# yatpor/bpc_baseline

Measured on AMD Instinct MI355X. Metric: detection-pairs matched/sec, higher is better.
Workload: dtype f64

## Files before the change

### bpc_baseline_amd/_native.py

```python
from __future__ import annotations

import ctypes
import os
import re

PKG_DIR = os.path.dirname(os.path.abspath(__file__))
LIB_PATH = os.environ.get("MVM_LIB_PATH") or os.path.join(PKG_DIR, "lib", "libmvmatch.so")
HEADER_PATH = os.path.join(os.path.dirname(PKG_DIR), "include", "mvmatch.h")

MVM_OK = 0
MVM_MAX_CAMS = 8
MVM_MAX_PAIRS = 28
MVM_F32, MVM_F64 = 0, 1

PAIRWISE_ARGMIN = {"default": 0, "lazy_transposed": 1, "lazy_rows": 2, "eager": 3}
CUBE_KERNEL = {"default": 0, "small": 1, "fused": 2, "workspace": 3, "generic": 4}


class MvmOptions(ctypes.Structure):
    _fields_ = [(n, ctypes.c_int32) for n in (
        "size", "pairwise_argmin", "pairwise_rows_per_wave", "pairwise_row_groups",
        "cube_kernel", "cube_rows_per_instr", "lsap_wave_max_cols", "lsap_multi_g",
        "lsap_lds_max_cols", "lsap_lds_small_cols", "lsap_mid_max_cols", "lsap_reg_max_cols",
        "lsap_reg_threads", "lsap_mreg_max_cols", "pairwise_row_interleave",
        "cube_cols_per_lane", "pairwise_xcd_fronts", "lsap_sparse_min_cols",
        "lsap_sparse_blocks", "cube_tile_rows")]


OPTION_FIELDS = [n for n, _ in MvmOptions._fields_[1:]]


def make_options(**kw):
    if not kw:
        return None
    o = MvmOptions()
    o.size = ctypes.sizeof(MvmOptions)
    for k, v in kw.items():
        if k not in OPTION_FIELDS:
            raise ValueError(f"unknown mvm_options field {k!r}")
        if k == "pairwise_argmin" and isinstance(v, str):
            v = PAIRWISE_ARGMIN[v]
        if k == "cube_kernel" and isinstance(v, str):
            v = CUBE_KERNEL[v]
        setattr(o, k, int(v))
    return o


class MvmError(RuntimeError):

    def __init__(self, fn: str, status: int, message: str):
        super().__init__(f"{fn} failed with status {status}: {message}")
        self.status = status


_vp = ctypes.c_void_p
_i32 = ctypes.c_int32
_i64 = ctypes.c_int64
_sz = ctypes.c_size_t

SIGNATURES = {
    "mvm_version": (ctypes.c_char_p, []),
    "mvm_last_error_string": (ctypes.c_char_p, []),
    "mvm_status_string": (ctypes.c_char_p, [ctypes.c_int]),
    "mvm_options_init": (None, [_vp]),
    "mvm_pairwise_residual_argmin": (ctypes.c_int, [
        _vp, _vp, _vp, _vp, _vp,
        _i32, _i32, _i32, _i32,
        _vp, _vp, _vp, _vp, _vp,
        _vp]),
    "mvm_pairwise_residual_argmin_ex": (ctypes.c_int, [
        _vp, _vp, _vp, _vp, _vp,
        _i32, _i32, _i32, _i32,
        _vp, _vp, _vp, _vp, _vp,
        _vp, _vp]),
    "mvm_pairwise_residual_argmin_pitched": (ctypes.c_int, [
        _vp, _vp, _vp, _vp, _vp,
        _i32, _i32, _i32, _i32, _i32,
        _vp, _vp, _vp, _vp, _vp,
        _vp, _vp]),
    "mvm_pairwise_residual_f64": (ctypes.c_int, [
        _vp, _vp, _vp, _vp, _vp,
        _i32, _i32, _i32, _i32,
        _i64, _i64, _vp,
        _vp]),
    "mvm_triplet_workspace_bytes": (_sz, [_i32, _i32]),
    "mvm_triplet_cost_argmin": (ctypes.c_int, [
        _vp, _vp, _vp, _i32, _i32,
        _vp, _vp, _vp, _vp, _vp,
        _vp, _sz, _vp]),
    "mvm_triplet_cost_argmin_ex": (ctypes.c_int, [
        _vp, _vp, _vp, _i32, _i32,
        _vp, _vp, _vp, _vp, _vp,
        _vp, _sz, _vp, _vp]),
    "mvm_triplet_cost_argmin_bmin8": (ctypes.c_int, [
        _vp, _vp, _vp, _i32, _i32,
        _vp, _vp, _vp, _vp, _vp,
        _vp, _vp,
        _vp, _sz, _vp, _vp]),
    "mvm_triplet_minima": (ctypes.c_int, [
        _vp, _vp, _vp, _i32, _i32,
        _vp, _vp, _vp, _vp,
        _vp, _sz, _vp, _vp]),
    "mvm_lsap_plan": (_i64, [_i32, _vp, _vp, _vp, _vp]),
    "mvm_lsap_plan_ex": (_i64, [_i32, _vp, _vp, _i32, _vp, _vp]),
    "mvm_lsap_solve": (ctypes.c_int, [
        _vp, _vp, _vp, _i32, _vp, _vp,
        _vp, _sz, _vp, _vp, _vp, _vp]),
    "mvm_lsap_solve_bounded": (ctypes.c_int, [
        _vp, _vp, _vp, _i32, _vp, _vp,
        _vp, _sz, _vp, _vp, _vp,
        _i64, _i64, _vp]),
    "mvm_lsap_solve_ex": (ctypes.c_int, [
        _vp, _i32, _vp, _vp, _i32, _vp, _vp,
        _vp, _sz, _vp, _vp, _vp,
        _i64, _i64, _vp, _vp]),
    "mvm_lsap_solve_ex2": (ctypes.c_int, [
        _vp, _i32, _vp, _vp, _i32, _vp, _vp,
        _vp, _sz, _vp, _vp, _vp,
        _i64, _i64, _i64, _vp, _vp]),
    "mvm_lsap_solve_ex3": (ctypes.c_int, [
        _vp, _i32, _vp, _vp, _i32, _vp, _vp,
        _vp, _sz, _vp, _vp, _vp,
        _i64, _i64, _i64,
        _vp, _vp, _vp, _vp, _vp]),
    "mvm_lsap_plan_resid": (_i64, [_i32, _vp, _vp, _vp, _vp]),
    "mvm_lsap_sparse_bounds": (None, [_vp, _vp, _vp]),
    "mvm_lsap_sparse_stats_offset": (_i64, [_i64, _i64]),
    "mvm_lsap_solve_resid": (ctypes.c_int, [
        _vp, _i32, _vp, _vp,
        _vp, _sz, _vp, _vp, _vp,
        _i64, _i64, _i64,
        _vp, _vp, _vp, _vp, _vp,
        _vp, _i32, _vp, _vp]),
    "mvm_pack_detections": (ctypes.c_int, [
        _vp, _vp, _vp, _vp, _i32,
        ctypes.c_float, ctypes.c_float,
        _vp, _vp, _vp, _vp, _vp, _vp]),
    "mvm_triangulate_dlt": (ctypes.c_int, [
        _vp, _vp, _vp, _i32, _i32, _vp, _vp]),
    "mvm_select_triangulate": (ctypes.c_int, [
        _vp, _vp, _vp, _vp, _vp, _vp,
        _vp, _vp, _i32, ctypes.c_double,
        _vp, _vp, _vp, _vp, _vp]),
    "mvm_select_triangulate_resid": (ctypes.c_int, [
        _vp, _i32, _vp, _vp, _vp, _vp,
        _vp, _vp, _i32, ctypes.c_double,
        _vp, _vp, _vp, _vp, _vp]),
    "mvm_compact_matches": (ctypes.c_int, [
        _vp, _vp, _vp, _vp, _vp,
        _vp, _vp, _vp, _i32, _i32,
        _vp, _vp, _vp, _vp, _vp, _vp, _vp,
        _vp]),
    "mvm_rig_matrices": (ctypes.c_int, [
        _vp, _vp, _vp, _vp,
        _i32, _i32, _i32,
        _vp, _vp, _vp, _vp]),
    "mvm_hbm_write_probe": (ctypes.c_int, [_vp, _sz, _vp]),
}

_lib = None


def header_symbols() -> list:
    with open(HEADER_PATH) as fh:
        text = fh.read()
    return re.findall(r"^\s*(?:const\s+)?[a-z_0-9]+\s*\*?\s*(mvm_[a-z_0-9]+)\s*\(", text, re.M)


def load(path: str = LIB_PATH):
    global _lib
    if _lib is not None:
        return _lib
    if not os.path.exists(path):
        raise ImportError(
            f"{path} not found: build the HIP library first "
            "(python -c 'import __graft_entry__ as g; g.build()')")
    lib = ctypes.CDLL(path)
    for name, (res, args) in SIGNATURES.items():
        fn = getattr(lib, name)
        fn.restype = res
# ... 14 lines not shown
```

### bpc_baseline_amd/csrc/mvm_lsap_sparse.h

```cpp
#pragma once

#include <hip/hip_runtime.h>
#include <stdint.h>

#include "mvmatch.h"

constexpr int kSpMaxCols = 65536;
constexpr int kSpMaxShort = 1024;
constexpr int kSpBlock = 32;
constexpr int kSpTB = 16;
constexpr int kSpLCap = 128;
constexpr int kSpTileCols = 2048;
constexpr int kSparseMinCols = 4096;
constexpr int kWaveMaxCols = 1024;

struct LsapIo {
    const void *cost;
    const int64_t *cost_offs;
    const int64_t *dims;
    const int64_t *ws_offs;
    unsigned char *ws;
    const int64_t *out_offs;
    int64_t *row_ind;
    int64_t *col_ind;
    int32_t *status;
};

struct LsapSparseArgs : LsapIo {
    int32_t lo;
    int32_t wave_max;
    int32_t s_cap;
    const uint16_t *bmin8;
    const int64_t *bmin8_offs;
    const int64_t *segs;
    int32_t tb;
    const double *resid = nullptr;
    int64_t resid_stride = 0;
    int32_t resid_ld = 0;
    int32_t resid_rows = 0;
    const uint16_t *bm32 = nullptr;
    const int64_t *bm32_offs = nullptr;
};

constexpr int32_t kSpStatusBounds = 4;

constexpr int kSpMaxBlocks = 2048;

__host__ __device__ inline int lsap_sparse_seg(const LsapSparseArgs &a, int p, bool tr, int L) {
    if (((!a.bmin8 || !a.bmin8_offs) && !a.bm32) || !a.segs || !tr) return 0;
    const int64_t seg = a.segs[p];
    if (seg <= 0 || L % seg != 0) return 0;
    return (L / seg) * ((seg + 31) / 32) <= kSpMaxBlocks ? (int)seg : 0;
}

__host__ __device__ inline bool lsap_sparse_class(int32_t lo, int32_t wave_max, int64_t R, int64_t K) {
    const int64_t lng = R > K ? R : K, sht = R > K ? K : R;
    return lo > 0 && lng >= lo && lng > wave_max && lng <= kSpMaxCols && sht >= 1 && sht <= kSpMaxShort;
}

struct SpLayout {
    size_t stats, flags, bm, lcol, lval, ln, theta, total;
};
constexpr int kSpStats = 4;

__host__ __device__ inline SpLayout lsap_sparse_layout(int64_t S, int64_t L, size_t elem, bool tr,
                                                       bool ext_bm = false) {
    SpLayout y;
    size_t o = 0;
    auto take = [&](size_t bytes) {
        const size_t at = o;
        o += (bytes + 255) & ~(size_t)255;
        return at;
    };
    const int64_t nbf = (L + kSpBlock - 1) / kSpBlock, nbs = L < kSpMaxBlocks ? L : kSpMaxBlocks;
    const int64_t nb = tr && nbs > nbf ? nbs : nbf;
    const int64_t nt = (L + kSpTileCols - 1) / kSpTileCols;
    y.stats = take(kSpStats * 4);
    y.flags = take((size_t)(nt > 32 ? nt : 32) * 4);
    y.bm = take(ext_bm ? 0 : (size_t)S * nb * elem);
    y.lcol = take((size_t)S * kSpLCap * 4);
    y.lval = take((size_t)S * kSpLCap * elem);
    y.ln = take((size_t)S * 4);
    y.theta = take((size_t)S * elem);
    y.total = o;
    return y;
}

int lsap_sparse_launch_f32(const LsapSparseArgs &a, int32_t n, int64_t long_max, hipStream_t s);
int lsap_sparse_launch_f64(const LsapSparseArgs &a, int32_t n, int64_t long_max, hipStream_t s);
```

### bpc_baseline_amd/csrc/mvm_lsap_sparse.hip

```cpp
#include "mvm_lsap_sparse.h"

#include <math.h>
#include <stdint.h>

#include "mvm_device.h"
#include "mvm_internal.h"

#pragma clang fp contract(off)

namespace {

constexpr int kSpNT = 256;
constexpr int kSpRowGroups = 16;

template <typename CT>
struct SpKey;
template <>
struct SpKey<float> {
    using T = uint32_t;
    static constexpr T kMax = 0xFFFFFFFFu;
    __device__ static T of(float x) {
        const uint32_t b = __float_as_uint(x + 0.0f);
        return (b & 0x80000000u) ? ~b : (b | 0x80000000u);
    }
// ... 461 lines not shown
                if (c) {
                    const int pos = ng + sp_mbcnt(m);
                    if (pos < kSpLCap) s_grp[wave][pos] = e;
                }
                ng += __popcll(m);
            }
            __builtin_amdgcn_wave_barrier();
            nent = ng;
            eshift = 3;
            ent = s_grp[wave];
        }
        int cnt = kSpLCap + 1;
        if (nent <= kSpLCap) {
            cnt = 0;
            const int per = kWaveLanes >> eshift, emask = (1 << eshift) - 1;
            for (int m0 = 0; m0 < nent; m0 += 8 * per) {
                CT val[8];
                int col[8];
#pragma unroll
                for (int u = 0; u < 8; ++u) {
                    const int idx = m0 + u * per + (lane >> eshift);
                    const int cb = idx < nent ? ent[idx] : 0;
                    const int j = (cb & 0xFFFF) + (lane & emask);
                    col[u] = (lane & emask) < (cb >> 16) ? j : -1;
                    val[u] = col[u] >= 0 ? src.at(s, j) : (CT)0;
                }
#pragma unroll
                for (int u = 0; u < 8; ++u) {
                    const bool keep = col[u] >= 0 && val[u] <= theta;
                    const uint64_t m = __ballot(keep);
                    if (keep) {
                        const int pos = cnt + sp_mbcnt(m);
                        if (pos < kSpLCap) {
                            lcol[(int64_t)s * kSpLCap + pos] = col[u];
                            lval[(int64_t)s * kSpLCap + pos] = val[u];
                        }
                    }
                    cnt += __popcll(m);
                }
            }
        }
        __builtin_amdgcn_wave_barrier();
        if (lane == 0) {
            ln[s] = cnt <= kSpLCap ? cnt : -1;
            theta_out[s] = theta;
        }
    }
    if (ext) {
        bad = __syncthreads_or(bad);
        if (threadIdx.x == 0) reinterpret_cast<int32_t *>(ws + y.flags)[grp] = bad;
    }
}


struct SpRec {
    double a;
    double f;
    int32_t a_pos;
    int32_t a_q;
    int32_t a_ps;
    int32_t f_any;
    int32_t tail_q;
    uint32_t f_key;
};

__host__ __device__ inline size_t sp_solve_lds_bytes(int lw, int cap) {
    return (size_t)2 * lw * 4 + (size_t)8 * (cap + 4 * (cap + 1)) + (size_t)4 * (3 * cap + 5 * (cap + 1));
}

template <typename CT>
__device__ __forceinline__ double sp_block_min(double x, double *s_red, int wave) {
    x = wave_min_f64(x);
    if ((threadIdx.x & 63) == 0) s_red[wave] = x;
    __syncthreads();
    const double r = fmin(fmin(s_red[0], s_red[1]), fmin(s_red[2], s_red[3]));
    __syncthreads();
    return r;
}

__device__ __forceinline__ long long sp_block_max_i64(long long x, long long *s_red, int wave) {
    x = sp_wave_max_i64(x);
    if ((threadIdx.x & 63) == 0) s_red[wave] = x;
    __syncthreads();
    long long r = s_red[0];
    for (int w = 1; w < kSpNT / 64; ++w) r = s_red[w] > r ? s_red[w] : r;
    __syncthreads();
    return r;
}

template <typename CT, int KS>
__global__ __launch_bounds__(kSpNT) __attribute__((amdgpu_waves_per_eu(KS == 1 ? 4 : 1))) void sp_solve_kernel(LsapSparseArgs a, int32_t n, int32_t lw) {
    __shared__ SpRec s_rec[2][kSpNT / 64];
    __shared__ double s_redd[kSpNT / 64];
    __shared__ long long s_redl[kSpNT / 64];
    extern __shared__ __attribute__((aligned(16))) unsigned char s_dyn[];
    const int p = blockIdx.x;
    if (p >= n) return;
    const int64_t R = a.dims[2 * p], Kd = a.dims[2 * p + 1];
    if (R == 0 || Kd == 0) {
        if (threadIdx.x == 0) a.status[p] = 0;
        return;
    }
    if (!lsap_sparse_class(a.lo, a.wave_max, R, Kd)) {
        if (a.resid && threadIdx.x == 0) a.status[p] = kSpStatusBounds;
        return;
    }
    const bool tr = Kd < R;
    const int S = (int)(tr ? Kd : R), L = (int)(tr ? R : Kd);
    const int cap = a.s_cap;
    bool src_ok;
    const SpSrc<CT> src = sp_src<CT>(a, p, tr, S, L, lsap_sparse_seg(a, p, tr, L), src_ok);
    if (S > cap || L > 32 * lw || (KS == 1 && S > kSpNT) || !src_ok) {
        if (threadIdx.x == 0) a.status[p] = kSpStatusBounds;
        return;
    }
    const SpLayout y = lsap_sparse_layout(S, L, sizeof(CT), tr, a.bm32 != nullptr);
    const unsigned char *ws = a.ws + a.ws_offs[p];
    const int32_t *lcol = reinterpret_cast<const int32_t *>(ws + y.lcol);
    const CT *lval = reinterpret_cast<const CT *>(ws + y.lval);
    const int32_t *ln = reinterpret_cast<const int32_t *>(ws + y.ln);
    const CT *theta = reinterpret_cast<const CT *>(ws + y.theta);
    const int t = threadIdx.x, lane = t & 63, wave = t >> 6;

    uint32_t *s_asg = reinterpret_cast<uint32_t *>(s_dyn);
    uint32_t *s_mvb = s_asg + lw;
    double *s_u = reinterpret_cast<double *>(s_mvb + lw);
    double *s_m = s_u + cap;
    double *s_mp = s_m + cap + 1;
    double *s_f = s_mp + cap + 1;
    double *s_rb = s_f + cap + 1;
    int32_t *s_c4r = reinterpret_cast<int32_t *>(s_rb + cap + 1);
    int32_t *s_r4c = s_c4r + cap;
    int32_t *s_col = s_r4c + cap;
    int32_t *s_i = s_col + cap;
    int32_t *s_sl = s_i + cap + 1;
    int32_t *s_ps = s_sl + cap + 1;
    int32_t *s_mvc = s_ps + cap + 1;
    int32_t *s_mvp = s_mvc + cap + 1;

    {
        const int seg = lsap_sparse_seg(a, p, tr, L);
        const int nt = a.bm32 ? kSpRowGroups
                       : seg  ? ((L / seg) * ((seg + kSpBlock - 1) / kSpBlock) + 63) / 64
                              : (L + kSpTileCols - 1) / kSpTileCols;
        const int32_t *fl = reinterpret_cast<const int32_t *>(ws + y.flags);
        int bad = 0;
        for (int x = t; x < nt; x += kSpNT) bad |= fl[x];
        if (__syncthreads_or(bad)) {
            if (t == 0) a.status[p] = 1;
            return;
        }
    }
    __shared__ int s_novf;
    if (t == 0) s_novf = 0;
    int n_dense_min = 0, n_dense_tie = 0, n_steps = 0;
    for (int x = t; x < lw; x += kSpNT) {
        s_asg[x] = 0u;
        s_mvb[x] = 0u;
    }
    __syncthreads();
    {
        int ovf = 0;
// ... 334 lines not shown
                const int q = kk == k ? na : s_sl[kk];
                s_c4r[i2] = q;
                s_r4c[q] = i2;
                if (s == 0) break;
                kk = s - 1;
            }
        }
        __syncthreads();
    }
    if (t == 0) {
        int32_t *stt = reinterpret_cast<int32_t *>(a.ws + a.ws_offs[p] + y.stats);
        stt[0] = n_dense_min;
        stt[1] = n_dense_tie;
        stt[2] = s_novf;
        stt[3] = n_steps;
    }
    const int64_t o = a.out_offs[p];
    if (tr) {
        for (int kk = t; kk < S; kk += kSpNT) {
            const int rk = s_col[s_c4r[kk]];
            int rank = 0;
            for (int k2 = 0; k2 < S; ++k2) rank += s_col[s_c4r[k2]] < rk;
            a.row_ind[o + rank] = rk;
            a.col_ind[o + rank] = kk;
        }
    } else {
        for (int kk = t; kk < S; kk += kSpNT) {
            a.row_ind[o + kk] = kk;
            a.col_ind[o + kk] = s_col[s_c4r[kk]];
        }
    }
    if (t == 0) a.status[p] = 0;
}

template <typename CT>
int sp_launch(const LsapSparseArgs &a0, int32_t n, int64_t long_max, hipStream_t s) {
    LsapSparseArgs a = a0;
    const int64_t lmax = long_max < kSpMaxCols ? long_max : kSpMaxCols;
    const int tpp = (int)((lmax + kSpTileCols - 1) / kSpTileCols);
    if ((int64_t)n * tpp * kSpNT > 0xFFFFFFFFLL || (int64_t)n * kSpRowGroups * kSpNT > 0xFFFFFFFFLL ||
        (int64_t)n * (kSpMaxBlocks / 64) * kSpNT > 0xFFFFFFFFLL)
        return mvm_fail(MVM_ERR_UNSUPPORTED, "%d problems in one batch: split it", (int)n);
    if (sizeof(CT) != sizeof(float)) {
        a.bmin8 = nullptr;
        a.bmin8_offs = nullptr;
        a.segs = nullptr;
        a.resid = nullptr;
        a.bm32 = nullptr;
        a.bm32_offs = nullptr;
    }
    if (!a.resid) sp_blockmin_kernel<CT><<<dim3((unsigned)(n * tpp)), dim3(kSpNT), 0, s>>>(a, n, tpp);
    if (a.bmin8 && !a.bm32)
        sp_bmin8_reduce_kernel<<<dim3((unsigned)(n * (kSpMaxBlocks / 64))), dim3(kSpNT), 0, s>>>(a, n);
    if (sizeof(CT) == 4 && a.bm32)
        sp_lists_kernel<CT, sizeof(CT) == 4><<<dim3((unsigned)(n * kSpRowGroups)), dim3(kSpNT), 0, s>>>(a, n);
    else
        sp_lists_kernel<CT, false><<<dim3((unsigned)(n * kSpRowGroups)), dim3(kSpNT), 0, s>>>(a, n);
    const int cap = a.s_cap;
    const int lw = (int)(((lmax + 63) / 64) * 2);
    const size_t lds = sp_solve_lds_bytes(lw, cap);
    void (*kern)(LsapSparseArgs, int32_t, int32_t) = cap <= kSpNT ? sp_solve_kernel<CT, 1> : sp_solve_kernel<CT, 4>;
    if (const int st = mvm_raise_dynamic_lds(reinterpret_cast<const void *>(kern), lds)) return st;
    kern<<<dim3((unsigned)n), dim3(kSpNT), lds, s>>>(a, n, lw);
    return mvm_check_launch("lsap_sparse");
}

}

int lsap_sparse_launch_f32(const LsapSparseArgs &a, int32_t n, int64_t long_max, hipStream_t s) {
    return sp_launch<float>(a, n, long_max, s);
}

int lsap_sparse_launch_f64(const LsapSparseArgs &a, int32_t n, int64_t long_max, hipStream_t s) {
    return sp_launch<double>(a, n, long_max, s);
}

extern "C" {

int64_t mvm_lsap_sparse_stats_offset(int64_t rows, int64_t cols) {
    const bool tr = cols < rows;
    return (int64_t)lsap_sparse_layout(tr ? cols : rows, tr ? rows : cols, sizeof(float), tr).stats;
}

void mvm_lsap_sparse_bounds(int32_t *min_cols, int32_t *max_cols, int32_t *max_short) {
    if (min_cols) *min_cols = kSparseMinCols;
    if (max_cols) *max_cols = kSpMaxCols;
    if (max_short) *max_short = kSpMaxShort;
}

int64_t mvm_lsap_plan_resid(int32_t n_problems, const int64_t *rows, const int64_t *cols,
                            int64_t *ws_offs, int64_t *out_offs) {
    if (n_problems < 0 || (n_problems > 0 && (!rows || !cols || !ws_offs || !out_offs))) {
        mvm_set_error("mvm_lsap_plan_resid: invalid arguments");
        return -1;
    }
    const auto need = [](int64_t nr, int64_t nc, bool tr, size_t elem) {
        if (nc > kSpMaxCols || nr > kSpMaxShort) return (int64_t)0;
        return (int64_t)lsap_sparse_layout(nr, nc, elem, tr, true).total;
    };
    return mvm_lsap_plan_offsets("mvm_lsap_plan_resid", n_problems, rows, cols, sizeof(float), need,
                                 ws_offs, out_offs);
}

int mvm_lsap_solve_resid(const int64_t *dims_dev, int32_t n_problems, const int64_t *ws_offs_dev,
                         const int64_t *out_offs_dev, void *workspace_dev, size_t workspace_bytes,
                         int64_t *row_ind_dev, int64_t *col_ind_dev, int32_t *status_dev,
                         int64_t long_min, int64_t long_max, int64_t short_max,
                         const uint16_t *bmin8_dev, const int64_t *bmin8_offs_dev,
                         const uint16_t *bm32_dev, const int64_t *bm32_offs_dev,
                         const int64_t *segs_dev, const double *resid_dev, int32_t max_n,
                         const mvm_options *opts, mvm_stream_t stream) {
    mvm_clear_error();
    mvm_options o;
    int st = mvm_resolve_options(opts, o);
    if (st) return st;
    if (o.lsap_sparse_blocks < 0 || o.lsap_sparse_blocks > 64)
        return mvm_fail(MVM_ERR_INVALID_ARGUMENT, "lsap_sparse_blocks %d not in 0..64",
                        (int)o.lsap_sparse_blocks);
    if (n_problems < 0) return mvm_fail(MVM_ERR_INVALID_ARGUMENT, "negative n_problems");
    if (n_problems == 0) return MVM_OK;
    if (!dims_dev || !ws_offs_dev || !out_offs_dev || !status_dev)
        return mvm_fail(MVM_ERR_INVALID_ARGUMENT, "null pointer");
    const bool data_null = (bmin8_dev && !bmin8_offs_dev) || !bm32_dev || !bm32_offs_dev || !segs_dev ||
                           !resid_dev || !workspace_dev || !row_ind_dev || !col_ind_dev;
    if (max_n < 0 || max_n > kChunk)
        return mvm_fail(MVM_ERR_UNSUPPORTED, "mvm_lsap_solve_resid: views of at most %d detections "
                        "(max_n %d)", kChunk, (int)max_n);
    const int sp_lo = mvm_resolve_limit(o.lsap_sparse_min_cols, kSparseMinCols, INT32_MAX);
    const int wave_max = mvm_resolve_limit(o.lsap_wave_max_cols, kWaveMaxCols, kWaveMaxCols);
    if (long_max >= 1) {
        if (sp_lo <= 0 || long_min < sp_lo || long_min <= wave_max || long_max > kSpMaxCols ||
            short_max < 1 || short_max > kSpMaxShort)
            return mvm_fail(MVM_ERR_INVALID_ARGUMENT,
                            "mvm_lsap_solve_resid: long sides [%lld, %lld] / short sides <= %lld are not "
                            "all of the candidate-list class (long sides >= %d, > %d, <= %d; short sides "
                            "<= %d)", (long long)long_min, (long long)long_max, (long long)short_max, sp_lo,
                            wave_max, kSpMaxCols, kSpMaxShort);
        if (data_null) return mvm_fail(MVM_ERR_INVALID_ARGUMENT, "null pointer");
    }
    (void)workspace_bytes;
    LsapSparseArgs sa{};
    sa.dims = dims_dev;
    sa.ws_offs = ws_offs_dev;
    sa.ws = reinterpret_cast<unsigned char *>(workspace_dev);
    sa.out_offs = out_offs_dev;
    sa.row_ind = row_ind_dev;
    sa.col_ind = col_ind_dev;
    sa.status = status_dev;
    sa.lo = sp_lo > 0 ? sp_lo : 1;
    sa.wave_max = wave_max;
    sa.s_cap = (int32_t)(short_max < 1 ? 1 : short_max);
    sa.bmin8 = bmin8_dev;
    sa.bmin8_offs = bmin8_dev ? bmin8_offs_dev : nullptr;
    sa.segs = segs_dev;
    sa.tb = o.lsap_sparse_blocks ? o.lsap_sparse_blocks : kSpTB;
    const int ld = (max_n + 3) / 4 * 4;
    sa.resid = resid_dev;
    sa.resid_ld = ld;
    sa.resid_rows = max_n;
    sa.resid_stride = (int64_t)3 * max_n * ld;
    sa.bm32 = bm32_dev;
    sa.bm32_offs = bm32_offs_dev;
    return sp_launch<float>(sa, n_problems, long_max < 1 ? 1 : long_max,
                            reinterpret_cast<hipStream_t>(stream));
}

}
```

### bpc_baseline_amd/ops.py

```python
from __future__ import annotations

import ctypes
from typing import List, Optional, Tuple

import numpy as np
import torch
from torch import Tensor

from . import _native

__all__ = [
    "PairwisePlan", "TripletPlan",
    "pairwise_residual_argmin", "pairwise_residual_f64", "triplet_cost_argmin",
    "hbm_write_probe", "LsapPlan", "linear_sum_assignment_batched",
    "pack_detections", "triangulate_dlt", "select_triangulate",
    "triplet_minima", "linear_sum_assignment_resid", "select_triangulate_resid",
    "cube_free_scenes", "sparse_class_bounds", "lsap_sparse_stats", "compact_matches",
    "rig_matrices",
]


def _h2d_int64(arrays: List[np.ndarray], device: torch.device) -> List[Tensor]:
    flat = np.concatenate([np.ascontiguousarray(a, dtype=np.int64).reshape(-1) for a in arrays])
    host = torch.from_numpy(flat)
    if device.type == "cuda":
        dev = host.pin_memory().to(device, non_blocking=True)
    else:
        dev = host.to(device)
    out, o = [], 0
    for a in arrays:
        out.append(dev[o:o + a.size])
        o += a.size
    return out


def _opts_list(options: Optional[dict]) -> Optional[List[int]]:
    o = _native.make_options(**(options or {}))
    return None if o is None else [int(getattr(o, n)) for n in _native.OPTION_FIELDS]


def _opts_ref(opts: Optional[List[int]]):
    if opts is None:
        return None
    if len(opts) != len(_native.OPTION_FIELDS):
        raise ValueError(f"opts: expected {len(_native.OPTION_FIELDS)} values, got {len(opts)}")
    return ctypes.byref(_native.make_options(**dict(zip(_native.OPTION_FIELDS, opts))))


def _p(t: Optional[Tensor]):
    if t is None or t.numel() == 0:
        return None
    return ctypes.c_void_p(t.data_ptr())


def _stream(t: Tensor):
    return ctypes.c_void_p(torch.cuda.current_stream(t.device).cuda_stream)


def _require(t: Tensor, name: str, dtype: torch.dtype, device: torch.device) -> None:
    if t.dtype != dtype:
        raise ValueError(f"{name}: expected {dtype}, got {t.dtype}")
    if t.device != device:
        raise ValueError(f"{name}: expected device {device}, got {t.device}")
    if not t.is_contiguous():
        raise ValueError(f"{name}: must be contiguous")


def _check_inputs(pts: Tensor, cam_offs: Tensor, F: Tensor, n_views: int, n_mats: int) -> None:
    if pts.device.type != "cuda":
        raise ValueError("pts must be a GPU tensor (the matcher has no CPU path)")
# ... 653 lines not shown
        self.out_offs_host = out_offs
        self.device = torch.device(device)
        self.dims, self.ws_offs, self.out_offs = _h2d_int64(
            [np.stack([rows, cols], axis=1).reshape(-1), ws_offs, out_offs], self.device)
        self.workspace = torch.empty(max(int(total), 16), dtype=torch.uint8, device=self.device)
        self.n_out = int(out_offs[-1])
        longs = np.maximum(rows, cols)[(rows > 0) & (cols > 0)]
        self.long_min = int(longs.min()) if longs.size else 0
        self.long_max = int(longs.max()) if longs.size else 0
        shorts = np.minimum(rows, cols)[(rows > 0) & (cols > 0)]
        self.short_max = int(shorts.max()) if shorts.size else 0


def linear_sum_assignment_batched(cost: Tensor, cost_offs: Tensor, plan: LsapPlan, *,
                                  options: Optional[dict] = None,
                                  bmin8: Optional[Tuple[Tensor, Tensor, Tensor]] = None):
    if cost.dtype != plan.dtype:
        raise ValueError(f"cost is {cost.dtype} but the plan was built for {plan.dtype}")
    dev = cost.device
    row_ind = torch.empty(max(plan.n_out, 1), dtype=torch.int64, device=dev)
    col_ind = torch.empty(max(plan.n_out, 1), dtype=torch.int64, device=dev)
    status = torch.empty(plan.n, dtype=torch.int32, device=dev)
    if bmin8 is not None and cost.dtype == torch.float32:
        torch.ops.mvmatch.lsap_solve_bmin8_out(cost, cost_offs, plan.dims, plan.ws_offs, plan.out_offs,
                                               plan.workspace, row_ind, col_ind, status, bmin8[0],
                                               bmin8[1], bmin8[2], plan.long_min, plan.long_max,
                                               plan.short_max, _opts_list(options))
        return row_ind[:plan.n_out], col_ind[:plan.n_out], status
    torch.ops.mvmatch.lsap_solve_out(cost, cost_offs, plan.dims, plan.ws_offs, plan.out_offs,
                                     plan.workspace, row_ind, col_ind, status, plan.long_min,
                                     plan.long_max, _opts_list(options), plan.short_max)
    return row_ind[:plan.n_out], col_ind[:plan.n_out], status


def lsap_sparse_stats(plan: LsapPlan, min_cols: Optional[int] = None) -> np.ndarray:
    lib = _native.load()
    lo, hi, sh = sparse_class_bounds()
    lo = lo if min_cols is None else int(min_cols)
    lng, sht = np.maximum(plan.rows, plan.cols), np.minimum(plan.rows, plan.cols)
    cls = (lng >= lo) & (lng > 1024) & (lng <= hi) & (sht >= 1) & (sht <= sh)
    out = np.full((plan.n, 4), -1, np.int64)
    if not cls.any():
        return out
    ps = np.nonzero(cls)[0]
    offs = np.array([plan.ws_offs_host[p] + lib.mvm_lsap_sparse_stats_offset(int(plan.rows[p]),
                                                                             int(plan.cols[p]))
                     for p in ps], np.int64)
    idx = torch.from_numpy((offs[:, None] // 4 + np.arange(4)).reshape(-1)).to(plan.workspace.device)
    words = plan.workspace[:plan.workspace.numel() // 4 * 4].view(torch.int32)
    out[ps] = words.index_select(0, idx).cpu().numpy().reshape(-1, 4)
    return out


def linear_sum_assignment_resid(plan: LsapPlan, tplan: TripletPlan, minima, *,
                                options: Optional[dict] = None):
    if not plan.resid:
        raise ValueError("linear_sum_assignment_resid needs LsapPlan(..., resid=True)")
    bmin8, bm32 = minima
    dev = bm32.device
    row_ind = torch.empty(max(plan.n_out, 1), dtype=torch.int64, device=dev)
    col_ind = torch.empty(max(plan.n_out, 1), dtype=torch.int64, device=dev)
    status = torch.empty(plan.n, dtype=torch.int32, device=dev)
    torch.ops.mvmatch.lsap_solve_resid_out(plan.dims, plan.ws_offs, plan.out_offs, plan.workspace,
                                           row_ind, col_ind, status, bmin8, tplan.bmin8_offs, bm32,
                                           tplan.bm32_offs, tplan.segs, tplan.workspace, tplan.max_n,
                                           plan.long_min, plan.long_max, plan.short_max,
                                           _opts_list(options))
    return row_ind[:plan.n_out], col_ind[:plan.n_out], status


def pack_detections(boxes: Tensor, conf: Tensor, cls: Tensor, img_offs: Tensor,
                    conf_thresh: float, class_id: float = 0.0):
    dev = boxes.device
    n = int(boxes.shape[0])
    n_img = int(img_offs.numel()) - 1
    counts = torch.empty(max(n_img, 0), dtype=torch.int32, device=dev)
    cam_offs = torch.zeros(max(n_img, 0) + 1, dtype=torch.int64, device=dev)
    pts = torch.empty((n, 2), dtype=torch.float64, device=dev)
    boxes_out = torch.empty((n, 4), dtype=torch.int32, device=dev)
    status = torch.zeros(1, dtype=torch.int32, device=dev)
    thresh = float(np.float32(conf_thresh))
    torch.ops.mvmatch.pack_detections_out(boxes.contiguous(), conf.contiguous(), cls.contiguous(),
                                          img_offs, thresh, float(np.float32(class_id)), counts,
                                          cam_offs, pts, boxes_out, status)
    return pts, cam_offs, boxes_out, counts, status


def triangulate_dlt(proj: Tensor, pts2d: Tensor, set_of_point: Optional[Tensor] = None) -> Tensor:
    X = torch.empty((int(pts2d.shape[0]), 3), dtype=torch.float64, device=pts2d.device)
    torch.ops.mvmatch.triangulate_dlt_out(proj.contiguous(), set_of_point, pts2d.contiguous(), X)
    return X


def select_triangulate(cube: Tensor, cube_offs: Tensor, cam_offs: Tensor, lsap_offs: Tensor,
                       row_ind: Tensor, col_ind: Tensor, pts: Tensor, proj: Tensor,
                       threshold: float):
    dev = cube.device
    cap = int(row_ind.numel())
    n_scenes = int(lsap_offs.numel()) - 1
    match = torch.empty((cap, 3), dtype=torch.int32, device=dev)
    cost = torch.empty(cap, dtype=torch.float32, device=dev)
    X = torch.empty((cap, 3), dtype=torch.float64, device=dev)
    count = torch.empty(n_scenes, dtype=torch.int32, device=dev)
    torch.ops.mvmatch.select_triangulate_out(cube, cube_offs, cam_offs, lsap_offs, row_ind,
                                             col_ind, pts, proj.contiguous(), float(threshold),
                                             match, cost, X, count)
# ... 84 lines not shown
```

### include/mvmatch.h

```cpp
#ifndef MVMATCH_H
#define MVMATCH_H

#include <stddef.h>
#include <stdint.h>

#ifdef __cplusplus
extern "C" {
#endif

#define MVM_ABI_VERSION 8
#define MVM_HAS_RIG_MATRICES 1
#define MVM_MAX_CAMS 8
#define MVM_MAX_PAIRS 28

typedef struct ihipStream_t *mvm_stream_t;

enum {
    MVM_OK = 0,
    MVM_ERR_INVALID_ARGUMENT = 1,
    MVM_ERR_UNSUPPORTED = 2,
    MVM_ERR_WORKSPACE = 3,
    MVM_ERR_HIP = 4
};

enum { MVM_F32 = 0, MVM_F64 = 1 };

const char *mvm_version(void);
const char *mvm_last_error_string(void);
const char *mvm_status_string(int status);

enum {
    MVM_PAIRWISE_ARGMIN_DEFAULT = 0,
    MVM_PAIRWISE_ARGMIN_LAZY_TRANSPOSED,
    MVM_PAIRWISE_ARGMIN_LAZY_ROWS,
    MVM_PAIRWISE_ARGMIN_EAGER
};
enum {
    MVM_CUBE_DEFAULT = 0,
    MVM_CUBE_SMALL,
    MVM_CUBE_FUSED,
    MVM_CUBE_WORKSPACE,
    MVM_CUBE_GENERIC
};
typedef struct mvm_options {
    int32_t size;
    int32_t pairwise_argmin;
    int32_t pairwise_rows_per_wave;
    int32_t pairwise_row_groups;
    int32_t cube_kernel;
    int32_t cube_rows_per_instr;
    int32_t lsap_wave_max_cols;
    int32_t lsap_multi_g;
    int32_t lsap_lds_max_cols;
    int32_t lsap_lds_small_cols;
    int32_t lsap_mid_max_cols;
    int32_t lsap_reg_max_cols;
    int32_t lsap_reg_threads;
    int32_t lsap_mreg_max_cols;
    int32_t pairwise_row_interleave;
    int32_t cube_cols_per_lane;
    int32_t pairwise_xcd_fronts;
    int32_t lsap_sparse_min_cols;
    int32_t lsap_sparse_blocks;
    int32_t cube_tile_rows;
} mvm_options;

void mvm_options_init(mvm_options *opts);

int mvm_pairwise_residual_argmin(const double *pts_dev, const int64_t *cam_offs_dev,
                                 const double *F_dev, const int32_t *pair_a,
                                 const int32_t *pair_b, int32_t n_scenes, int32_t n_cams,
                                 int32_t n_pairs, int32_t max_n, const int64_t *dist_offs_dev,
                                 const int64_t *row_offs_dev, float *dist_dev,
                                 int32_t *argmin_dev, float *minval_dev, mvm_stream_t stream);
int mvm_pairwise_residual_argmin_ex(const double *pts_dev, const int64_t *cam_offs_dev,
                                    const double *F_dev, const int32_t *pair_a,
                                    const int32_t *pair_b, int32_t n_scenes, int32_t n_cams,
                                    int32_t n_pairs, int32_t max_n, const int64_t *dist_offs_dev,
                                    const int64_t *row_offs_dev, float *dist_dev,
                                    int32_t *argmin_dev, float *minval_dev,
                                    const mvm_options *opts, mvm_stream_t stream);

int mvm_pairwise_residual_argmin_pitched(const double *pts_dev, const int64_t *cam_offs_dev,
                                         const double *F_dev, const int32_t *pair_a,
                                         const int32_t *pair_b, int32_t n_scenes, int32_t n_cams,
                                         int32_t n_pairs, int32_t max_n, int32_t row_align,
                                         const int64_t *dist_offs_dev, const int64_t *row_offs_dev,
                                         float *dist_dev, int32_t *argmin_dev, float *minval_dev,
                                         const mvm_options *opts, mvm_stream_t stream);

int mvm_pairwise_residual_f64(const double *pts_dev, const int64_t *cam_offs_dev,
                              const double *F_dev, const int32_t *pair_a, const int32_t *pair_b,
                              int32_t n_scenes, int32_t n_cams, int32_t n_pairs,
                              int32_t max_n, int64_t mat_stride, int64_t ld, double *e_dev,
                              mvm_stream_t stream);

size_t mvm_triplet_workspace_bytes(int32_t n_scenes, int32_t max_n);
int mvm_triplet_cost_argmin(const double *pts_dev, const int64_t *cam_offs_dev,
                            const double *F_dev, int32_t n_scenes, int32_t max_n,
                            const int64_t *cube_offs_dev, const int64_t *row_offs_dev,
                            float *cube_dev, int32_t *argmin_dev, float *minval_dev,
                            void *workspace_dev, size_t workspace_bytes, mvm_stream_t stream);
int mvm_triplet_cost_argmin_ex(const double *pts_dev, const int64_t *cam_offs_dev,
                               const double *F_dev, int32_t n_scenes, int32_t max_n,
                               const int64_t *cube_offs_dev, const int64_t *row_offs_dev,
                               float *cube_dev, int32_t *argmin_dev, float *minval_dev,
                               void *workspace_dev, size_t workspace_bytes,
                               const mvm_options *opts, mvm_stream_t stream);
int mvm_triplet_cost_argmin_bmin8(const double *pts_dev, const int64_t *cam_offs_dev,
                                  const double *F_dev, int32_t n_scenes, int32_t max_n,
                                  const int64_t *cube_offs_dev, const int64_t *row_offs_dev,
                                  float *cube_dev, int32_t *argmin_dev, float *minval_dev,
                                  uint16_t *bmin8_dev, const int64_t *bmin8_offs_dev,
                                  void *workspace_dev, size_t workspace_bytes,
                                  const mvm_options *opts, mvm_stream_t stream);

int mvm_triplet_minima(const double *pts_dev, const int64_t *cam_offs_dev, const double *F_dev,
                       int32_t n_scenes, int32_t max_n, uint16_t *bmin8_dev,
                       const int64_t *bmin8_offs_dev, uint16_t *bm32_dev, const int64_t *bm32_offs_dev,
                       double *resid_dev, size_t resid_bytes, const mvm_options *opts,
                       mvm_stream_t stream);

int64_t mvm_lsap_plan(int32_t n_problems, const int64_t *rows, const int64_t *cols,
                      int64_t *ws_offs, int64_t *out_offs);
int mvm_lsap_solve(const float *cost_dev, const int64_t *cost_offs_dev, const int64_t *dims_dev,
                   int32_t n_problems, const int64_t *ws_offs_dev, const int64_t *out_offs_dev,
                   void *workspace_dev, size_t workspace_bytes, int64_t *row_ind_dev,
                   int64_t *col_ind_dev, int32_t *status_dev, mvm_stream_t stream);
int mvm_lsap_solve_bounded(const float *cost_dev, const int64_t *cost_offs_dev,
                           const int64_t *dims_dev, int32_t n_problems,
                           const int64_t *ws_offs_dev, const int64_t *out_offs_dev,
                           void *workspace_dev, size_t workspace_bytes, int64_t *row_ind_dev,
                           int64_t *col_ind_dev, int32_t *status_dev, int64_t long_min,
                           int64_t long_max, mvm_stream_t stream);
int64_t mvm_lsap_plan_ex(int32_t n_problems, const int64_t *rows, const int64_t *cols,
                         int32_t cost_dtype, int64_t *ws_offs, int64_t *out_offs);
int mvm_lsap_solve_ex(const void *cost_dev, int32_t cost_dtype, const int64_t *cost_offs_dev,
                      const int64_t *dims_dev, int32_t n_problems, const int64_t *ws_offs_dev,
                      const int64_t *out_offs_dev, void *workspace_dev, size_t workspace_bytes,
                      int64_t *row_ind_dev, int64_t *col_ind_dev, int32_t *status_dev,
                      int64_t long_min, int64_t long_max, const mvm_options *opts,
                      mvm_stream_t stream);
int mvm_lsap_solve_ex2(const void *cost_dev, int32_t cost_dtype, const int64_t *cost_offs_dev,
                       const int64_t *dims_dev, int32_t n_problems, const int64_t *ws_offs_dev,
                       const int64_t *out_offs_dev, void *workspace_dev, size_t workspace_bytes,
                       int64_t *row_ind_dev, int64_t *col_ind_dev, int32_t *status_dev,
                       int64_t long_min, int64_t long_max, int64_t short_max,
                       const mvm_options *opts, mvm_stream_t stream);
int mvm_lsap_solve_ex3(const void *cost_dev, int32_t cost_dtype, const int64_t *cost_offs_dev,
                       const int64_t *dims_dev, int32_t n_problems, const int64_t *ws_offs_dev,
                       const int64_t *out_offs_dev, void *workspace_dev, size_t workspace_bytes,
                       int64_t *row_ind_dev, int64_t *col_ind_dev, int32_t *status_dev,
                       int64_t long_min, int64_t long_max, int64_t short_max,
                       const uint16_t *bmin8_dev, const int64_t *bmin8_offs_dev,
                       const int64_t *segs_dev, const mvm_options *opts, mvm_stream_t stream);

int64_t mvm_lsap_plan_resid(int32_t n_problems, const int64_t *rows, const int64_t *cols,
                            int64_t *ws_offs, int64_t *out_offs);
void mvm_lsap_sparse_bounds(int32_t *min_cols, int32_t *max_cols, int32_t *max_short);
int64_t mvm_lsap_sparse_stats_offset(int64_t rows, int64_t cols);
int mvm_lsap_solve_resid(const int64_t *dims_dev, int32_t n_problems, const int64_t *ws_offs_dev,
                         const int64_t *out_offs_dev, void *workspace_dev, size_t workspace_bytes,
                         int64_t *row_ind_dev, int64_t *col_ind_dev, int32_t *status_dev,
                         int64_t long_min, int64_t long_max, int64_t short_max,
                         const uint16_t *bmin8_dev, const int64_t *bmin8_offs_dev,
                         const uint16_t *bm32_dev, const int64_t *bm32_offs_dev,
                         const int64_t *segs_dev, const double *resid_dev, int32_t max_n,
                         const mvm_options *opts, mvm_stream_t stream);

int mvm_pack_detections(const float *boxes_dev, const float *conf_dev, const float *cls_dev,
                        const int64_t *img_offs_dev, int32_t n_img, float conf_thresh,
                        float class_id, int32_t *counts_dev, int64_t *cam_offs_dev,
                        double *pts_dev, int32_t *boxes_out_dev, int32_t *status_dev,
                        mvm_stream_t stream);

int mvm_triangulate_dlt(const double *proj_dev, const int32_t *set_of_point_dev,
                        const double *pts2d_dev, int32_t n_points, int32_t n_views, double *X_dev,
                        mvm_stream_t stream);

int mvm_select_triangulate(const float *cube_dev, const int64_t *cube_offs_dev,
                           const int64_t *cam_offs_dev, const int64_t *lsap_out_offs_dev,
                           const int64_t *row_ind_dev, const int64_t *col_ind_dev,
                           const double *pts_dev, const double *proj_dev, int32_t n_scenes,
                           double threshold, int32_t *match_dev, float *cost_dev, double *X_dev,
                           int32_t *count_dev, mvm_stream_t stream);
int mvm_select_triangulate_resid(const double *resid_dev, int32_t max_n, const int64_t *cam_offs_dev,
                                 const int64_t *lsap_out_offs_dev, const int64_t *row_ind_dev,
                                 const int64_t *col_ind_dev, const double *pts_dev,
                                 const double *proj_dev, int32_t n_scenes, double threshold,
                                 int32_t *match_dev, float *cost_dev, double *X_dev, int32_t *count_dev,
                                 mvm_stream_t stream);

int mvm_compact_matches(const int32_t *match_dev, const float *cost_dev, const double *X_dev,
                        const int32_t *count_dev, const int64_t *seg_offs_dev, const double *pts_dev,
                        const int32_t *boxes_dev, const int64_t *cam_offs_dev, int32_t n_scenes,
                        int32_t scene_base, int64_t *dense_offs_dev, int32_t *scene_out_dev,
                        int32_t *match_out_dev, float *cost_out_dev, double *X_out_dev,
                        int32_t *boxes_out_dev, double *cent_out_dev, mvm_stream_t stream);

int mvm_rig_matrices(const float *K_dev, const double *RT_dev, const int32_t *pair_a,
                     const int32_t *pair_b, int32_t n_scenes, int32_t n_cams, int32_t n_pairs,
                     double *F_dev, double *proj_dev, int32_t *status_dev, mvm_stream_t stream);

int mvm_hbm_write_probe(void *dst_dev, size_t bytes, mvm_stream_t stream);

#ifdef __cplusplus
}
#endif

#endif
```

Measured before the change: 1613 billion.

## Add wave-per-row sparse candidate list kernel for resid float LSAP path

Adds a new sp_lists_ext_kernel that processes two rows per wave, loading bm32 keys with vectorized loads and staging the row's e13/e23 residual slices in LDS. It does a per-row ballot binary search for the threshold and compacts candidate blocks before evaluating cube costs. It becomes the default for the resid float path, with an option to fall back to the previous list kernel. It also zeroes stats in-kernel, short-circuits to a status memset when no problems are in the sparse class, adds a debug accessor for the lists, and drops the long_max clamp. The aim is to cut list-building cost through more memory-level parallelism and fewer redundant global loads, at the price of a 4-waves-per-EU cap and extra LDS per workgroup.

```diff
diff --git a/bpc_baseline_amd/_native.py b/bpc_baseline_amd/_native.py
--- a/bpc_baseline_amd/_native.py
+++ b/bpc_baseline_amd/_native.py
@@ -24,7 +24,7 @@
         "lsap_lds_max_cols", "lsap_lds_small_cols", "lsap_mid_max_cols", "lsap_reg_max_cols",
         "lsap_reg_threads", "lsap_mreg_max_cols", "pairwise_row_interleave",
         "cube_cols_per_lane", "pairwise_xcd_fronts", "lsap_sparse_min_cols",
-        "lsap_sparse_blocks", "cube_tile_rows")]
+        "lsap_sparse_blocks", "cube_tile_rows", "lsap_sparse_lists")]
 
 
 OPTION_FIELDS = [n for n, _ in MvmOptions._fields_[1:]]
@@ -126,6 +126,7 @@
     "mvm_lsap_plan_resid": (_i64, [_i32, _vp, _vp, _vp, _vp]),
     "mvm_lsap_sparse_bounds": (None, [_vp, _vp, _vp]),
     "mvm_lsap_sparse_stats_offset": (_i64, [_i64, _i64]),
+    "mvm_lsap_sparse_list_offsets": (_i32, [_i64, _i64, _i32, _vp]),
     "mvm_lsap_solve_resid": (ctypes.c_int, [
         _vp, _i32, _vp, _vp,
         _vp, _sz, _vp, _vp, _vp,
diff --git a/bpc_baseline_amd/csrc/mvm_lsap_sparse.h b/bpc_baseline_amd/csrc/mvm_lsap_sparse.h
--- a/bpc_baseline_amd/csrc/mvm_lsap_sparse.h
+++ b/bpc_baseline_amd/csrc/mvm_lsap_sparse.h
@@ -40,6 +40,7 @@
     int32_t resid_rows = 0;
     const uint16_t *bm32 = nullptr;
     const int64_t *bm32_offs = nullptr;
+    int32_t lists_prev = 0;
 };
 
 constexpr int32_t kSpStatusBounds = 4;
diff --git a/bpc_baseline_amd/csrc/mvm_lsap_sparse.hip b/bpc_baseline_amd/csrc/mvm_lsap_sparse.hip
--- a/bpc_baseline_amd/csrc/mvm_lsap_sparse.hip
+++ b/bpc_baseline_amd/csrc/mvm_lsap_sparse.hip
@@ -537,6 +537,208 @@
     }
 }
 
+constexpr int kSpExtRows = 2;
+constexpr int kSpExtRd = kChunk;
+typedef unsigned short sp_u16x2 __attribute__((ext_vector_type(2)));
+
+struct SpExtLds {
+    double rd[kSpNT / 64][kSpExtRows][2][kSpExtRd];
+    int32_t cand[kSpNT / 64][kSpExtRows * kSpLCap];
+};
+static_assert(4 * sizeof(SpExtLds) <= 160 * 1024, "four workgroups per CU: four waves per SIMD");
+
+__global__ __launch_bounds__(kSpNT) __attribute__((amdgpu_waves_per_eu(4, 4))) void sp_lists_ext_kernel(
+    LsapSparseArgs a, int32_t n) {
+    using K = SpKey<float>;
+    constexpr int kQ = kSpMaxCols / kSpBlock / 64;
+    constexpr int kW = kQ / 2;
+    constexpr int kRowStep = kSpRowGroups * (kSpNT / 64);
+    static_assert(kQ == 32, "32 keys per lane");
+    __shared__ SpExtLds sm;
+    const int p = (int)(blockIdx.x / kSpRowGroups), grp = (int)(blockIdx.x % kSpRowGroups);
+    if (p >= n) return;
+    const int64_t R = a.dims[2 * p], Kd = a.dims[2 * p + 1];
+    if (!lsap_sparse_class(a.lo, a.wave_max, R, Kd)) return;
+    const bool tr = Kd < R;
+    const int S = (int)(tr ? Kd : R), L = (int)(tr ? R : Kd);
+    const SpLayout y = lsap_sparse_layout(S, L, sizeof(float), tr, true);
+    unsigned char *ws = a.ws + a.ws_offs[p];
+    int32_t *lcol = reinterpret_cast<int32_t *>(ws + y.lcol);
+    float *lval = reinterpret_cast<float *>(ws + y.lval);
+    int32_t *ln = reinterpret_cast<int32_t *>(ws + y.ln);
+    float *theta_out = reinterpret_cast<float *>(ws + y.theta);
+    const int seg = lsap_sparse_seg(a, p, tr, L);
+    bool src_ok;
+    const SpSrc<float> src = sp_src<float>(a, p, tr, S, L, seg, src_ok);
+    if (!src_ok || !seg) return;
+    const int bps = (seg + kSpBlock - 1) / kSpBlock, nseg = L / seg;
+    const int nb = nseg * bps;
+    const int npad = (nseg + 15) & ~15;
+    const int rowk = npad * bps;
+    const float rnpad = 1.0f / (float)npad;
+    const int kpl = (rowk + 63) >> 6;
+    const int ld = src.ld;
+    const bool fits = ld <= kSpExtRd && nseg <= ld && seg <= ld;
+    const int wave = threadIdx.x / 64, lane = threadIdx.x % 64;
+    const uint16_t *bm16 = a.bm32 + a.bm32_offs[p];
+    int32_t *cand = sm.cand[wave];
+    int bad = 0;
+    for (int s0 = grp * (kSpNT / 64) + wave; s0 < S; s0 += kSpExtRows * kRowStep) {
+        uint32_t kp[kSpExtRows][kW];
+        double2 st[kSpExtRows][2][2];
+#pragma unroll
+        for (int r = 0; r < kSpExtRows; ++r) {
+            const int64_t s_u = __builtin_amdgcn_readfirstlane(s0 + r * kRowStep);
+            const bool live = s_u < S;
+            const uint16_t *row16 = bm16 + s_u * rowk;
+            if (!live) {
+#pragma unroll
+                for (int w = 0; w < kW; ++w) kp[r][w] = 0xFFFFFFFFu;
+            } else if (kpl == 32) {
+                const uint4 *r4 = reinterpret_cast<const uint4 *>(row16) + 4 * lane;
+#pragma unroll
+                for (int v = 0; v < 4; ++v) {
+                    const uint4 w = r4[v];
+                    kp[r][4 * v] = w.x;
+                    kp[r][4 * v + 1] = w.y;
+                    kp[r][4 * v + 2] = w.z;
+                    kp[r][4 * v + 3] = w.w;
+                }
+            } else {
+                const uint16_t *lp = row16 + kpl * lane;
+                const int nk = min(kpl, rowk - kpl * lane);
+#pragma unroll
+                for (int w = 0; w < kW; ++w) {
+                    const uint32_t h0 = 2 * w < nk ? (uint32_t)lp[2 * w] : 0xFFFFu;
+                    const uint32_t h1 = 2 * w + 1 < nk ? (uint32_t)lp[2 * w + 1] : 0xFFFFu;
+                    kp[r][w] = h0 | (h1 << 16);
+                }
+            }
+#pragma unroll
+            for (int m = 0; m < 2; ++m) {
+                const double *row = (m ? src.e23t : src.e13t) + s_u * ld;
+#pragma unroll
+                for (int h = 0; h < 2; ++h) {
+                    const int x = 2 * lane + 128 * h;
+                    st[r][m][h] = live && fits && x < ld ? *reinterpret_cast<const double2 *>(row + x)
+                                                         : make_double2(0.0, 0.0);
+                }
+            }
+        }
+        uint32_t lh[kSpExtRows];
+#pragma unroll
+        for (int r = 0; r < kSpExtRows; ++r) {
+            sp_u16x2 m2 = __builtin_bit_cast(sp_u16x2, kp[r][0]);
+#pragma unroll
+            for (int w = 1; w < kW; ++w)
+                m2 = __builtin_elementwise_min(m2, __builtin_bit_cast(sp_u16x2, kp[r][w]));
+            const uint32_t mh = min((uint32_t)m2.x, (uint32_t)m2.y);
+            bad |= mh < 0x8000u;
+            lh[r] = mh == 0xFFFFu ? 0xFFFFu : min(mh, 0xFF80u);
+        }
+        uint32_t lo[kSpExtRows], hi[kSpExtRows];
+#pragma unroll
+        for (int r = 0; r < kSpExtRows; ++r) {
+            lo[r] = 0;
+            hi[r] = 0xFFFFu;
+        }
+        if (nb > a.tb) {
+            for (int it = 0; it < 16; ++it) {
+#pragma unroll
+                for (int r = 0; r < kSpExtRows; ++r) {
+                    const uint32_t mid = lo[r] + (hi[r] - lo[r]) / 2;
+                    if (__popcll(__ballot(lh[r] <= mid)) >= a.tb) hi[r] = mid;
+                    else lo[r] = mid + 1;
+                }
+            }
+        }
+#pragma unroll
+        for (int r = 0; r < kSpExtRows; ++r)
+#pragma unroll
+            for (int m = 0; m < 2; ++m)
+#pragma unroll
+                for (int h = 0; h < 2; ++h)
+                    *reinterpret_cast<double2 *>(&sm.rd[wave][r][m][2 * lane + 128 * h]) = st[r][m][h];
+        float theta[kSpExtRows];
+        int ncand[kSpExtRows];
+#pragma unroll
+        for (int r = 0; r < kSpExtRows; ++r) {
+            theta[r] = (float)INFINITY;
+            uint32_t cut = 0xFFFEu;
+            if (nb > a.tb) {
+                theta[r] = K::val((lo[r] << 16) | 0xFFFFu);
+                cut = lo[r] >= 0xFF80u ? 0xFFFEu : lo[r];
+            }
+            int nc = 0;
+#pragma unroll
+            for (int q = 0; q < kQ; ++q) {
+                const uint32_t h = (q & 1) ? kp[r][q >> 1] >> 16 : kp[r][q >> 1] & 0xFFFFu;
+                const bool c = h <= cut;
+                const uint64_t m = __ballot(c);
+                if (m) {
+                    if (c) {
+                        const int pos = nc + sp_mbcnt(m);
+                        if (pos < kSpLCap) {
+                            int g;
+                            const int jt = sp_div(kpl * lane + q, npad, rnpad, g);
+                            cand[r * kSpLCap + pos] = g | (jt << 12);
+                        }
+                    }
+                    nc += __popcll(m);
+                }
+            }
+            ncand[r] = nc;
+        }
+        __builtin_amdgcn_wave_barrier();
+        const int n0 = fits && ncand[0] <= kSpLCap ? ncand[0] : 0;
+        const int n1 = fits && ncand[1] <= kSpLCap ? ncand[1] : 0;
+        const int nent = n0 + n1;
+        int cnt0 = 0, cnt1 = 0;
+        const int l32 = lane & 31;
+        for (int m0 = 0; m0 < nent; m0 += 16) {
+            double e12[8], e13[8], e23[8];
+            int col[8];
+#pragma unroll
+            for (int u = 0; u < 8; ++u) {
+                const int idx = m0 + 2 * u + (lane >> 5);
+                const bool in0 = idx < n0;
+                const int e = idx < nent ? cand[in0 ? idx : kSpLCap + idx - n0] : 0;
+                const int g = e & 0xFFF, jj = (e >> 12) * kSpBlock + l32;
+                const bool ok = idx < nent && jj < seg;
+                col[u] = ok ? g * seg + jj : -1;
+                e12[u] = ok ? src.e12[g * ld + jj] : 0.0;
+                e13[u] = ok ? sm.rd[wave][in0 ? 0 : 1][0][g] : 0.0;
+                e23[u] = ok ? sm.rd[wave][in0 ? 0 : 1][1][jj] : 0.0;
+            }
+#pragma unroll
+            for (int u = 0; u < 8; ++u) {
+                const bool in0 = m0 + 2 * u + (lane >> 5) < n0;
+                const float val = cube_f32(e12[u], e13[u], e23[u]);
+                const bool keep = col[u] >= 0 && val <= (in0 ? theta[0] : theta[1]);
+                const uint64_t k0 = __ballot(keep && in0), k1 = __ballot(keep && !in0);
+                if (keep) {
+                    const int pos = in0 ? cnt0 + sp_mbcnt(k0) : cnt1 + sp_mbcnt(k1);
+                    if (pos < kSpLCap) {
+                        const int64_t s = s0 + (in0 ? 0 : kRowStep);
+                        lcol[s * kSpLCap + pos] = col[u];
+                        lval[s * kSpLCap + pos] = val;
+                    }
+                }
+                cnt0 += __popcll(k0);
+                cnt1 += __popcll(k1);
+            }
+        }
+        __builtin_amdgcn_wave_barrier();
+        if (lane < kSpExtRows && s0 + lane * kRowStep < S) {
+            const int nc = lane ? ncand[1] : ncand[0], cnt = lane ? cnt1 : cnt0;
+            ln[s0 + lane * kRowStep] = fits && nc <= kSpLCap && cnt <= kSpLCap ? cnt : -1;
+            theta_out[s0 + lane * kRowStep] = lane ? theta[1] : theta[0];
+        }
+    }
+    bad = __syncthreads_or(bad);
+    if (threadIdx.x == 0) reinterpret_cast<int32_t *>(ws + y.flags)[grp] = bad;
+}
+
 
 struct SpRec {
     double a;
@@ -593,6 +795,11 @@
     const bool tr = Kd < R;
     const int S = (int)(tr ? Kd : R), L = (int)(tr ? R : Kd);
     const int cap = a.s_cap;
+    if (threadIdx.x == 0) {
+        int32_t *stt = reinterpret_cast<int32_t *>(
+            a.ws + a.ws_offs[p] + lsap_sparse_layout(S, L, sizeof(CT), tr, a.bm32 != nullptr).stats);
+        for (int x = 0; x < kSpStats; ++x) stt[x] = 0;
+    }
     bool src_ok;
     const SpSrc<CT> src = sp_src<CT>(a, p, tr, S, L, lsap_sparse_seg(a, p, tr, L), src_ok);
     if (S > cap || L > 32 * lw || (KS == 1 && S > kSpNT) || !src_ok) {
@@ -1033,7 +1240,10 @@
     if (!a.resid) sp_blockmin_kernel<CT><<<dim3((unsigned)(n * tpp)), dim3(kSpNT), 0, s>>>(a, n, tpp);
     if (a.bmin8 && !a.bm32)
         sp_bmin8_reduce_kernel<<<dim3((unsigned)(n * (kSpMaxBlocks / 64))), dim3(kSpNT), 0, s>>>(a, n);
-    if (sizeof(CT) == 4 && a.bm32)
+    if (sizeof(CT) == 4 && a.bm32 && a.resid && !a.bmin8 && !a.lists_prev &&
+        (reinterpret_cast<uintptr_t>(a.resid) & 15) == 0)
+        sp_lists_ext_kernel<<<dim3((unsigned)(n * kSpRowGroups)), dim3(kSpNT), 0, s>>>(a, n);
+    else if (sizeof(CT) == 4 && a.bm32)
         sp_lists_kernel<CT, sizeof(CT) == 4><<<dim3((unsigned)(n * kSpRowGroups)), dim3(kSpNT), 0, s>>>(a, n);
     else
         sp_lists_kernel<CT, false><<<dim3((unsigned)(n * kSpRowGroups)), dim3(kSpNT), 0, s>>>(a, n);
@@ -1061,6 +1271,20 @@
 int64_t mvm_lsap_sparse_stats_offset(int64_t rows, int64_t cols) {
     const bool tr = cols < rows;
     return (int64_t)lsap_sparse_layout(tr ? cols : rows, tr ? rows : cols, sizeof(float), tr).stats;
+}
+
+int mvm_lsap_sparse_list_offsets(int64_t rows, int64_t cols, int32_t resid, int64_t *offs) {
+    mvm_clear_error();
+    if (rows < 1 || cols < 1 || !offs)
+        return mvm_fail(MVM_ERR_INVALID_ARGUMENT, "mvm_lsap_sparse_list_offsets: invalid arguments");
+    const bool tr = cols < rows;
+    const SpLayout y = lsap_sparse_layout(tr ? cols : rows, tr ? rows : cols, sizeof(float), tr, resid != 0);
+    offs[0] = (int64_t)y.flags;
+    offs[1] = (int64_t)y.lcol;
+    offs[2] = (int64_t)y.lval;
+    offs[3] = (int64_t)y.ln;
+    offs[4] = (int64_t)y.theta;
+    return MVM_OK;
 }
 
 void mvm_lsap_sparse_bounds(int32_t *min_cols, int32_t *max_cols, int32_t *max_short) {
@@ -1098,6 +1322,8 @@
     if (o.lsap_sparse_blocks < 0 || o.lsap_sparse_blocks > 64)
         return mvm_fail(MVM_ERR_INVALID_ARGUMENT, "lsap_sparse_blocks %d not in 0..64",
                         (int)o.lsap_sparse_blocks);
+    if (o.lsap_sparse_lists < 0 || o.lsap_sparse_lists > 1)
+        return mvm_fail(MVM_ERR_INVALID_ARGUMENT, "lsap_sparse_lists %d not 0 or 1", (int)o.lsap_sparse_lists);
     if (n_problems < 0) return mvm_fail(MVM_ERR_INVALID_ARGUMENT, "negative n_problems");
     if (n_problems == 0) return MVM_OK;
     if (!dims_dev || !ws_offs_dev || !out_offs_dev || !status_dev)
@@ -1118,6 +1344,11 @@
                             "<= %d)", (long long)long_min, (long long)long_max, (long long)short_max, sp_lo,
                             wave_max, kSpMaxCols, kSpMaxShort);
         if (data_null) return mvm_fail(MVM_ERR_INVALID_ARGUMENT, "null pointer");
+    } else {
+        if (hipMemsetAsync(status_dev, 0, (size_t)n_problems * sizeof(int32_t),
+                           reinterpret_cast<hipStream_t>(stream)) != hipSuccess)
+            return mvm_fail(MVM_ERR_HIP, "mvm_lsap_solve_resid: cannot clear the statuses");
+        return MVM_OK;
     }
     (void)workspace_bytes;
     LsapSparseArgs sa{};
@@ -1142,7 +1373,8 @@
     sa.resid_stride = (int64_t)3 * max_n * ld;
     sa.bm32 = bm32_dev;
     sa.bm32_offs = bm32_offs_dev;
-    return sp_launch<float>(sa, n_problems, long_max < 1 ? 1 : long_max,
+    sa.lists_prev = o.lsap_sparse_lists;
+    return sp_launch<float>(sa, n_problems, long_max,
                             reinterpret_cast<hipStream_t>(stream));
 }
 
diff --git a/bpc_baseline_amd/ops.py b/bpc_baseline_amd/ops.py
--- a/bpc_baseline_amd/ops.py
+++ b/bpc_baseline_amd/ops.py
@@ -15,7 +15,7 @@
     "hbm_write_probe", "LsapPlan", "linear_sum_assignment_batched",
     "pack_detections", "triangulate_dlt", "select_triangulate",
     "triplet_minima", "linear_sum_assignment_resid", "select_triangulate_resid",
-    "cube_free_scenes", "sparse_class_bounds", "lsap_sparse_stats", "compact_matches",
+    "cube_free_scenes", "sparse_class_bounds", "lsap_sparse_stats", "lsap_sparse_lists", "compact_matches",
     "rig_matrices",
 ]
 
@@ -775,6 +775,29 @@
     return out
 
 
+def lsap_sparse_lists(plan: LsapPlan, p: int) -> dict:
+    if plan.dtype != torch.float32:
+        raise ValueError("lsap_sparse_lists: float32 plans only")
+    rows, cols = int(plan.rows[p]), int(plan.cols[p])
+    offs = (ctypes.c_int64 * 5)()
+    st = _native.load().mvm_lsap_sparse_list_offsets(rows, cols, int(plan.resid), offs)
+    _native.check("mvm_lsap_sparse_list_offsets", st)
+    short = min(rows, cols)
+    cap = 128
+    base = int(plan.ws_offs_host[p])
+
+    def take(off, count, dtype):
+        raw = plan.workspace[base + off:base + off + 4 * count].cpu().numpy()
+        return raw.view(dtype).copy()
+
+    n_flags = 16 if plan.resid else max((max(rows, cols) + 2047) // 2048, 32)
+    return {"flags": take(offs[0], n_flags, np.int32),
+            "lcol": take(offs[1], short * cap, np.int32).reshape(short, cap),
+            "lval": take(offs[2], short * cap, np.float32).reshape(short, cap),
+            "ln": take(offs[3], short, np.int32),
+            "theta": take(offs[4], short, np.float32)}
+
+
 def linear_sum_assignment_resid(plan: LsapPlan, tplan: TripletPlan, minima, *,
                                 options: Optional[dict] = None):
     if not plan.resid:
diff --git a/include/mvmatch.h b/include/mvmatch.h
--- a/include/mvmatch.h
+++ b/include/mvmatch.h
@@ -63,6 +63,7 @@
     int32_t lsap_sparse_min_cols;
     int32_t lsap_sparse_blocks;
     int32_t cube_tile_rows;
+    int32_t lsap_sparse_lists;
 } mvm_options;
 
 void mvm_options_init(mvm_options *opts);
@@ -159,6 +160,7 @@
                             int64_t *ws_offs, int64_t *out_offs);
 void mvm_lsap_sparse_bounds(int32_t *min_cols, int32_t *max_cols, int32_t *max_short);
 int64_t mvm_lsap_sparse_stats_offset(int64_t rows, int64_t cols);
+int mvm_lsap_sparse_list_offsets(int64_t rows, int64_t cols, int32_t resid, int64_t *offs);
 int mvm_lsap_solve_resid(const int64_t *dims_dev, int32_t n_problems, const int64_t *ws_offs_dev,
                          const int64_t *out_offs_dev, void *workspace_dev, size_t workspace_bytes,
                          int64_t *row_ind_dev, int64_t *col_ind_dev, int32_t *status_dev,
```

Result: no change. 1613 billion (-0.1%).
